# GadGadGad/Convolutional-KAN-for-Image-Classification

Hardware: AMD Instinct MI355X
Metric: images/sec fwd+bwd KAN-VGG11 3x32x32 bs=256/GPU (higher is better)
Workload: dtype f32

## Files before the change

convolutional-kan-for-image-classification_amd/_lib.py:

```python
from __future__ import annotations

import ctypes as C
import os
from typing import Optional

_HERE = os.path.dirname(os.path.abspath(__file__))
LIB_PATH = os.environ.get("KANCONV_LIB") or os.path.join(_HERE, "libkanconv.so")

KAN_MAX_PLANES = 16
KAN_MAX_TABLE = 32
KAN_FP_WORDS = 192
BASIS_BSPLINE, BASIS_RBF, BASIS_CHEBY, BASIS_POLY, BASIS_FOURIER, BASIS_RELU, BASIS_GRAM = 0, 1, 2, 3, 4, 5, 6
ACT_NONE, ACT_IDENTITY, ACT_GELU, ACT_SILU, ACT_RELU, ACT_TANH, ACT_SIGMOID, ACT_GELU_TANH = -1, 0, 1, 2, 3, 4, 5, 6
ORDER_QUAD_FWD, ORDER_ROWBLK8_FWD, ORDER_QUAD_BWD_DATA, ORDER_FWD_WEIGHT_SIDE = 1, 2, 4, 8


class KanGeom(C.Structure):
    _fields_ = [(n, C.c_int) for n in ("B", "C", "H", "W", "O", "Ho", "Wo", "kh", "kw", "sh", "sw", "ph", "pw", "dh", "dw", "groups")] + \
               [("x_bstride", C.c_longlong), ("y_bstride", C.c_longlong)]


class KanBasis(C.Structure):
    _fields_ = [("kind", C.c_int), ("n_basis", C.c_int), ("order", C.c_int), ("act", C.c_int),
                ("p0", C.c_float), ("p1", C.c_float), ("table", C.c_float * KAN_MAX_TABLE), ("chan_table", C.c_void_p)]


class KanPlan(C.Structure):
    _fields_ = [(n, C.c_int) for n in ("P", "K", "IPC", "KC", "Kpad", "Opad", "fwd_splits", "bwd_data_splits", "bwd_weight_splits",
                                          "fwd_target", "bwd_data_target", "bwd_weight_target", "x_pm_wanted", "dz_pm_wanted", "bwd_weight_expanded", "row_blocks", "e_pm_wanted", "fwd_expanded", "fwd_halo", "bwd_weight_halo",
                                          "fwd_band", "bwd_weight_band")] + \
               [(n, C.c_longlong) for n in ("packed_weight_bytes", "bwd_data_weight_bytes", "fwd_slab_elems", "bwd_data_slab_elems",
                                            "bwd_weight_slab_elems", "e_pm_elems")]


class KanNormRoute(C.Structure):
    _fields_ = [(n, C.c_int) for n in ("kernel", "G", "EPL", "PPI", "NT", "pool", "lds", "held", "blocks", "strided")]


NORM_GENERIC, NORM_REGS = 0, 1
NORM_POOL_NONE, NORM_POOL_2X2, NORM_POOL_K = 0, 1, 2


class KanWavGeom(C.Structure):
    _fields_ = [(n, C.c_int) for n in ("B", "C", "H", "W", "O", "Ho", "Wo", "kh", "kw", "sh", "sw", "ph", "pw", "dh", "dw", "wavelet")] + \
               [("x_bstride", C.c_longlong), ("u_bstride", C.c_longlong)]


class KanWavRoute(C.Structure):
    _fields_ = [(n, C.c_int) for n in ("TH", "TW", "NIMG", "RH", "RW", "tiles_h", "tiles_w", "fwd_shrunk", "fwd_nimg_cut", "fwd_lds_bytes", "fwd_fits",
                                       "fwd_blocks", "bwd_input_kernel", "bwd_input_blocks", "params_kernel", "passes", "chunks", "BH", "NI", "RU",
                                       "CU", "XP", "UP", "bands", "items", "items_per_chunk", "lds_bytes", "px_per_chunk")]


WAV_BI_TAPS9, WAV_BI_STRIDE1, WAV_BI_STRIDED = 0, 1, 2
WAV_PAR_TILED, WAV_PAR_PIXEL = 0, 1


WAVELETS = {"mexican_hat": 0, "morlet": 1, "dog": 2, "meyer": 3, "shannon": 4}

_P, _I, _LL, _F, _D = C.c_void_p, C.c_int, C.c_longlong, C.c_float, C.c_double
_GP, _BP = C.POINTER(KanGeom), C.POINTER(KanBasis)
SIGNATURES = {
    "kan_version": (C.c_char_p, []),
    "kan_last_error": (C.c_char_p, []),
    "kan_plan": (_I, [_GP, _BP, C.POINTER(KanPlan)]),
    "kan_tile_orders": (_I, [_GP, _BP]),
    "kan_pack_weights": (_I, [_P, _P, _P, _P, _GP, _BP, _P]),
    "kan_pack_weights_iod": (_I, [_P, _P, _P, _GP, _BP, _P]),
    "kan_pack_cacheable": (_I, [_GP, _BP]),
    "kan_pack_weights_cached": (_I, [_P, _P, _P, _P, _GP, _BP, _P, _I, _I, _I, _P]),
    "kan_conv_fwd": (_I, [_P, _P, _P, _P, _GP, _BP, _P, _P]),
    "kan_position_major": (_I, [_P, _P, _I, _I, _I, _LL, _P]),
    "kan_conv_bwd_data": (_I, [_P, _P, _P, _P, _P, _P, _GP, _BP, _P, _P]),
    "kan_conv_bwd_data_params": (_I, [_P, _P, _P, _P, _P, _P, _P, _GP, _BP, _P, _P]),
    "kan_conv_bwd_weight": (_I, [_P, _P, _P, _P, _GP, _BP, _P, _P, _P]),
    "kan_position_major_expanded": (_I, [_P, _P, _GP, _BP, _P]),
    "kan_conv_fwd_expanded": (_I, [_P, _P, _P, _GP, _BP, _P]),
    "kan_conv_fwd_expanded_order": (_I, [_P, _P, _P, _GP, _BP, _P, _I]),
    "kan_conv_bwd_weight_expanded": (_I, [_P, _P, _P, _GP, _BP, _P]),
    "kan_unpack_wgrad": (_I, [_P, _P, _P, _GP, _BP, _P]),
    "kan_unpack_wgrad_iod": (_I, [_P, _P, _GP, _BP, _P]),
    "kan_slab_reduce": (_I, [_P, _I, _LL, _P, _I, _I, _I, _LL, _P]),
    "kan_instnorm_prelu_fwd": (_I, [_P, _I, _LL, _P, _P, _P, _P, _P, _P, _P, _I, _I, _I, _LL, _F, _I, _P]),
    "kan_instnorm_prelu_bwd": (_I, [_P, _P, _P, _P, _P, _P, _P, _P, _P, _P, _P, _I, _I, _I, _LL, _I, _P]),
    "kan_instnorm_prelu_pool_fwd": (_I, [_P, _I, _LL, _P, _P, _P, _P, _P, _P, _P, _P, _I, _I, _I, _I, _LL, _F, _I, _P]),
    "kan_instnorm_prelu_pool_bwd": (_I, [_P, _P, _P, _P, _P, _P, _P, _P, _P, _P, _P, _P, _I, _I, _I, _I, _LL, _I, _P]),
    "kan_instnorm_prelu_poolk_fwd": (_I, [_P, _I, _LL, _P, _P, _P, _P, _P, _P, _P, _P, _I, _I, _I, _I, _LL, _F, _I, _I, _I, _P]),
    "kan_instnorm_prelu_poolk_bwd": (_I, [_P, _P, _P, _P, _P, _P, _P, _P, _P, _P, _P, _P, _I, _I, _I, _I, _LL, _I, _I, _I, _P]),
    "kan_norm_route": (_I, [_I, _I, _I, _I, _I, _LL, _I, _LL, _I, _I, _I, _I, C.POINTER(KanNormRoute)]),
    "kan_batchnorm_workspace_bytes": (_LL, [_I, _I]),
    "kan_batchnorm_prelu_fwd": (_I, [_P, _I, _LL, _P, _P, _P, _P, _P, _P, _P, _P, _P, _P, _P, _I, _I, _I, _I, _LL, _F, _D, _I, _I, _P]),
    "kan_batchnorm_prelu_bwd": (_I, [_P, _P, _P, _P, _P, _P, _P, _P, _P, _P, _P, _P, _P, _I, _I, _I, _I, _LL, _I, _I, _P]),
    "kan_split_supported": (_I, [C.POINTER(KanGeom), C.POINTER(KanBasis)]),
    "kan_split_weight_bytes": (_LL, [C.POINTER(KanGeom), C.POINTER(KanBasis)]),
    "kan_split_pack_weights": (_I, [_P, _P, _P, C.POINTER(KanGeom), C.POINTER(KanBasis), _P]),
    "kan_conv_fwd_split": (_I, [_P, _P, _P, C.POINTER(KanGeom), C.POINTER(KanBasis), _P]),
    "kan_split_bwd_data_weight_bytes": (_LL, [C.POINTER(KanGeom), C.POINTER(KanBasis)]),
    "kan_split_pack_weights_bwd_data": (_I, [_P, _P, _P, C.POINTER(KanGeom), C.POINTER(KanBasis), _P]),
    "kan_conv_bwd_data_split": (_I, [_P, _P, _P, _P, C.POINTER(KanGeom), C.POINTER(KanBasis), _P]),
    "kan_split_bwd_weight_workspace_bytes": (_LL, [C.POINTER(KanGeom), C.POINTER(KanBasis)]),
    "kan_conv_bwd_weight_split": (_I, [_P, _P, _P, _P, _P, C.POINTER(KanGeom), C.POINTER(KanBasis), _P]),
    "kan_wav_fwd": (_I, [_P, _P, _P, _P, _P, C.POINTER(KanWavGeom), _P]),
    "kan_wav_bwd_input": (_I, [_P, _P, _P, _P, _P, _P, C.POINTER(KanWavGeom), _P]),
    "kan_wav_param_workspace": (_LL, [C.POINTER(KanWavGeom)]),
    "kan_wav_bwd_params": (_I, [_P, _P, _P, _P, _P, _P, _P, _P, _P, C.POINTER(KanWavGeom), _P]),
    "kan_wav_route": (_I, [C.POINTER(KanWavGeom), C.POINTER(KanWavRoute)]),
    "kan_adamw_step": (_I, [_P, _P, _P, _P, _LL, _D, _D, _D, _D, _D, _I, _F, _P]),
    "kan_adamw_step_segments": (_I, [_P, _P, _P, _P, _P, _P, _P, _P, _P, _I, _I, _D, _D, _D, _D, _D, _I, _F, _P]),
    "kan_adamw_advance": (_I, [_P, _P, _I, _P]),
    "kan_adamw_step_segments_dev": (_I, [_P, _P, _P, _P, _P, _P, _P, _P, _P, _P, _I, _I, _D, _D, _D, _D, _F, _P]),
    "kan_adamw_dev_args": (_I, [_P, _P, _D, _D, _D, _D, _F, _P, _P]),
    "kan_grad_sqnorm_chunks": (_I, [_P, _P, _P, _P, _I, _I, _P, _P]),
# ... 48 lines not shown
```

convolutional-kan-for-image-classification_amd/csrc/kan_internal.h:

```cpp
#pragma once
#include <type_traits>
#include "kanconv.h"

int kan_fail_msg(const char* fmt, const char* a);
int kan_raise_lds_limit(const void* kernel, int bytes);

enum : int {
    FAST_GENERIC = 0,
    FAST_BSPLINE_SILU = 1,
    FAST_BSPLINE_GELU = 2,
    FAST_RBF8 = 3,
    FAST_CHEBY5 = 4,
    FAST_CHEBY4 = 5,
    FAST_POLY4 = 6,
    FAST_POLY3 = 7,
    FAST_RBF5 = 8,
    FAST_RELU8 = 9,
    FAST_GRAM4 = 10,
    FAST_POLY1 = 11,
    FAST_LAST = 11
};
enum : unsigned {
    ON_TAP_MAJOR = 1u << 0,
    ON_BIG_TILES = 1u << 1,
// ... 76 lines not shown
    unsigned char ph_a[KAN_BAND_MAX_PHASES], ph_b[KAN_BAND_MAX_PHASES];
    short ph_tap0[KAN_BAND_MAX_PHASES + 1];
    unsigned short tap_shift[KAN_BAND_MAX_TAPS];
    unsigned short tap_rt[KAN_BAND_MAX_TAPS];
    short tap_step[KAN_BAND_MAX_TAPS], tap_nt[KAN_BAND_MAX_TAPS];
} KanBandCfg;

void kan_band_cfg(const KanGeom* g, const KanBasis* b, int fast, KanBandCfg* cfg);
int kan_band_bwd_weight_launch(const float* dz, const float* x, const float* xn, float* dwp, const KanGeom* g, const KanBasis* b,
                               const KanBandCfg* cfg, int splits, long long slab_elems, void* stream);
int kan_band_fwd_launch(const float* x, const float* xn, const float* wp, float* z, const KanGeom* g, const KanBasis* b,
                        const KanBandCfg* cfg, int splits, long long slab_elems, void* stream);

constexpr int DW_T = 9;
constexpr int DW_MAX_TP = 96;

enum class Route { TAP_MAJOR, DW, BAND, HALO, EXPANDED };

struct FwdCfg { int TO, TP, tiles_o, tiles_p, chunks, splits, slots; };
struct BdCfg { int CH, tiles_c, tiles_p, n_ob, Opad32, chunks, splits; };
struct BwCfg { int TR, TO, tiles_r, tiles_o, chunks, splits, slots; };
struct BwHaloCfg { int R, nimg, spb, n_bands, tiles_r, tiles_o, splits, bands_per_split; };

struct ConvPlan {
    KanPlan pub;
    int fast;
    Route fwd, bwd_data, bwd_weight;
    bool pm_fwd, pm_bwd_data, pm_bwd_weight;
    bool rowblk_bwd_data;
    bool quad_fwd;
    bool quad_bd;
    bool rowblk8_fwd;
    bool fwd_wq;
    bool pmdma_xcd, pm_lpt, pm_xcd;
    FwdCfg fc;
    BdCfg bd;
    BwCfg bw;
    BwHaloCfg bwh;
    KanBandCfg band;
};
int plan_conv(const KanGeom* g, const KanBasis* b, ConvPlan* cp);

int live_taps_out(const KanGeom* g, int hw);
int live_taps_in(const KanGeom* g, int hw);
int live_positions_for_tap(const KanGeom* g, int tap);
int balance_tiles(const int* weight, int n, unsigned short* idx);
```

convolutional-kan-for-image-classification_amd/csrc/kan_plan.hip:

```cpp
#include <hip/hip_runtime.h>
#include <cstdio>
#include <cstdlib>
#include <cstring>
#include "kanconv.h"
#include "kan_device.h"
#include "kan_common.h"
#include "kan_internal.h"

namespace {

int fail(const char* msg) { return kan_fail_msg("%s", msg); }

int check(const KanGeom* g, const KanBasis* b) {
    if (!g || !b) return fail("null geometry/basis");
    if (g->groups < 0 || g->groups > 65535) return fail("groups out of range");
    if (g->B <= 0 || g->C <= 0 || g->O <= 0 || g->H <= 0 || g->W <= 0 || g->Ho <= 0 || g->Wo <= 0) return fail("non-positive dimension");
    if (g->kh <= 0 || g->kw <= 0 || g->sh <= 0 || g->sw <= 0 || g->dh <= 0 || g->dw <= 0 || g->ph < 0 || g->pw < 0) return fail("bad conv parameters");
    if (g->kh > 255 || g->kw > 255 || g->C > 65535) return fail("kernel size / channel count out of supported range");
    if ((g->H + 2 * g->ph - g->dh * (g->kh - 1) - 1) / g->sh + 1 != g->Ho || (g->W + 2 * g->pw - g->dw * (g->kw - 1) - 1) / g->sw + 1 != g->Wo)
        return fail("Ho/Wo inconsistent with H/W, kernel, stride, padding, dilation");
    if ((long long)g->B * g->Ho * g->Wo >= (1ll << 31) || (long long)g->B * g->H * g->W >= (1ll << 31)) return fail("pixel count exceeds int32");
    if ((long long)g->B * g->x_bstride * 4 >= (1ll << 31) || (long long)g->B * g->y_bstride * 4 >= (1ll << 31))
        return fail("activation tensors must be smaller than 2 GiB (32-bit buffer offsets)");
    if (g->x_bstride < (long long)ngroups(g) * g->C * g->H * g->W || g->y_bstride < (long long)ngroups(g) * g->O * g->Ho * g->Wo)
// ... 310 lines not shown
        const bool use18 = (long long)i18 * pl->P * 16 > (long long)i16 * pl->P * 18;
        pl->KC = use18 ? 18 : 16;
        pl->IPC = use18 ? i18 : i16;
        if (pl->P >= 10 && pl->P <= 12) { pl->KC = 12; pl->IPC = 1; }
        if (halo) { pl->KC = 2 * pl->P; pl->IPC = 2; }
    }
    pl->Kpad = ceil_div(g->C * T, pl->IPC) * pl->KC;
    if (band) { pl->KC = c.band.NPLE; pl->IPC = c.band.NG; pl->Kpad = c.band.n_steps * c.band.NPLE; }
    pl->Opad = round_up(g->O, 64);
    pl->packed_weight_bytes = (long long)G * pl->Kpad * pl->Opad * 4;
    c.bd = bd_cfg(g, *pl);
    pl->bwd_data_weight_bytes = (long long)G * T * c.bd.Opad32 * c.bd.tiles_c * 128 * 4;
    pl->fwd_slab_elems = (long long)g->B * g->y_bstride;
    pl->bwd_data_slab_elems = (long long)g->B * g->x_bstride;
    pl->bwd_weight_slab_elems = (long long)G * pl->K * pl->Opad;
    const bool big = big_tiles(f, *pl);
    c.fc = fwd_cfg(g, *pl, big, c.pm_fwd, halo);
    c.bw = bw_cfg(g, *pl, big, c.pm_bwd_weight);
    if (halo_bw) c.bwh = bw_halo_cfg(g, *pl);
    pl->fwd_splits = band ? c.band.fwd_splits : c.fc.splits;
    pl->bwd_data_splits = c.bd.splits;
    pl->bwd_weight_splits = halo_bw ? c.bwh.splits : c.bw.splits;
    if (band_bw) {
        pl->bwd_weight_splits = c.band.bw_splits;
        pl->bwd_weight_slab_elems = (long long)G * pl->Kpad * pl->Opad;
    }
    pl->fwd_target = pl->bwd_data_target = pl->bwd_weight_target = 0;
    const bool rowblk_fwd = halo && g->H == 4 && g->W == 4 && c.fc.TO == 256;
    c.quad_fwd = rowblk_fwd && g->B % 32 == 0 && !tuning_off("KAN_QUAD_FWD");
    c.quad_bd = c.rowblk_bwd_data && g->B % 32 == 0 && !tuning_off("KAN_QUAD_BD");
    c.rowblk8_fwd = halo && g->H == 8 && g->W == 8 && c.fc.TO == 256 && g->B % 4 == 0 && !tuning_off("KAN_ROWBLK8_FWD");
    c.fwd_wq = c.fwd == Route::EXPANDED && g->H == 2 && g->W == 2 && g->Ho == 2 && g->Wo == 2 && g->kh == 3 && g->kw == 3 && g->sh == 1 && g->sw == 1 &&
               g->ph == 1 && g->pw == 1 && g->dh == 1 && g->dw == 1 && pl->P == 9 && pl->KC == 18 && g->y_bstride % 4 == 0 && !tuning_off("KAN_PMDMA_FWD_WQ");
    if (dw) {
        pl->fwd_splits = pl->bwd_data_splits = 1;
        pl->bwd_weight_splits = dw_weight_chunks(g);
        pl->bwd_data_weight_bytes = pl->packed_weight_bytes;
        c.pm_fwd = c.pm_bwd_data = c.pm_bwd_weight = false;
    }
    if (c.pm_fwd) {
        LiveClass cls[16]; const int plane = g->Ho * g->Wo;
        const long long tiles_per_pos = (long long)ceil_div(g->B, c.fc.TP) * c.fc.tiles_o * G;
        for (int hw = 0; hw < plane; ++hw) cls[hw] = LiveClass{tiles_per_pos, live_taps_out(g, hw) * ceil_div(g->C, pl->IPC)};
        pl->fwd_target = pick_target_steps(cls, plane, 8, 4.0 * g->B * g->O * g->Ho * g->Wo * G, &pl->fwd_splits, c.fc.slots);
    }
    if (c.pm_bwd_weight) {
        LiveClass cw[32];
        const long long tiles_per_tap = (long long)ceil_div((long long)g->C * pl->P, c.bw.TR) * c.bw.tiles_o * G;
        for (int tap = 0; tap < T; ++tap) cw[tap] = LiveClass{tiles_per_tap, live_positions_for_tap(g, tap) * ceil_div(g->B, 16)};
        pl->bwd_weight_target = pick_target_steps(cw, T, 16, 4.0 * pl->K * pl->Opad * G, &pl->bwd_weight_splits, c.bw.slots);
    }
    if (c.pm_bwd_data) {
        LiveClass cls[16]; const int plane = g->H * g->W;
        const long long tiles_per_pos = (long long)ceil_div(g->B, 128) * c.bd.tiles_c * G;
        for (int hw = 0; hw < plane; ++hw) cls[hw] = LiveClass{tiles_per_pos, live_taps_in(g, hw) * c.bd.n_ob};
        pl->bwd_data_target = pick_target_steps(cls, plane, 8, 4.0 * g->B * g->C * g->H * g->W * G, &pl->bwd_data_splits);
    }
    pl->fwd_halo = c.fwd == Route::HALO;
    pl->fwd_band = c.fwd == Route::BAND;
    pl->fwd_expanded = c.fwd == Route::EXPANDED;
    pl->bwd_weight_halo = c.bwd_weight == Route::HALO;
    pl->bwd_weight_band = c.bwd_weight == Route::BAND;
    pl->bwd_weight_expanded = c.bwd_weight == Route::EXPANDED;
    pl->x_pm_wanted = (c.pm_fwd && c.fwd != Route::EXPANDED) || (c.pm_bwd_weight && c.bwd_weight != Route::EXPANDED);
    pl->dz_pm_wanted = c.pm_bwd_data || c.pm_bwd_weight;
    pl->e_pm_wanted = pl->fwd_expanded || pl->bwd_weight_expanded;
// ... 5 lines not shown
```

convolutional-kan-for-image-classification_amd/csrc/kanconv.hip:

```cpp
#include <hip/hip_runtime.h>
#include <cstdio>
#include <cstdlib>
#include <cstring>
#include <cmath>
#include <cstdint>
#include <mutex>
#include <type_traits>
#include <vector>
#include "kanconv.h"
#include "kan_device.h"

#include "kan_common.h"
#include "kan_internal.h"

namespace {


thread_local char g_err[512] = "";
int fail(const char* fmt, const char* a = "") {
    snprintf(g_err, sizeof(g_err), fmt, a);
    return -1;
}
}
int kan_fail_msg(const char* fmt, const char* a) { return fail(fmt, a); }
// ... 1281 lines not shown
    for (int cur = 0; ch < ch1; cur ^= 1) {
        stage(cur);
        __syncthreads();
        ch = next_live(ch + 1);
        if (ch < ch1) issue(ch);
        const float* cE = sE + cur * (KPX * LDE) + MRG;
        const float* cZ = sZ + cur * (KPX * LDZ);
        const unsigned ae = lds_addr(cE + kh2 * LDE + ar), az = lds_addr(cZ + kh2 * LDZ + bo);
        KAN_MFMA_STEP(KPX / 2, ae, LDE, az, LDZ);
    }

    float* out = dwp + (size_t)blk.z * slab_elems;
#pragma unroll
    for (int mi = 0; mi < 2; ++mi)
#pragma unroll
        for (int r = 0; r < 16; ++r) {
            const int row = k0 + w_r * 64 + mi * 32 + mfma_row(r, lane);
            if (row >= Krows) continue;
#pragma unroll
            for (int ni = 0; ni < 2; ++ni) {
                const int o = o_tile0 + w_c * 64 + ni * 32 + (lane & 31);
                out[(size_t)row * Opad + o] = acc[mi][ni][r];
            }
        }
}

#define LDS_READ4W(r0, r1, r2, r3, a0, a1, b, oA, oB0, oB1)                                                              \
    asm volatile("ds_read_b32 %0, %4 offset:%7\n\tds_read_b32 %1, %5 offset:%7\n\tds_read_b32 %2, %6 offset:%8\n\tds_read_b32 %3, %6 offset:%9" \
                 : "=&v"(r0), "=&v"(r1), "=&v"(r2), "=&v"(r3) : "v"(a0), "v"(a1), "v"(b), "n"(oA), "n"(oB0), "n"(oB1) : "memory")

template <int FAST, int W, int R, int NIMG>
__global__ __launch_bounds__(256, 4) void k_conv_bwd_weight_halo(
    const float* __restrict__ dz, const float* __restrict__ x, float* __restrict__ dwp, DevGeom g, DevBasis bs, int Krows, int Opad,
    int n_bands, int bands_per_split, long long slab_elems, unsigned x_bytes, unsigned dz_bytes, int tiles_o) {
    constexpr int KIND = fast_kind(FAST);
    constexpr int P = fast_planes(FAST), T = 9, PT = P * T;
    constexpr int TR = 128, TO = 128, NT = 256, KPX = 16;
    constexpr int HWc = W + 2, HIMG = (R + 2) * HWc, CELLS = NIMG * HIMG;
    constexpr int PS = W == 16 ? CELLS + 1 : W == 8 ? CELLS + 3 : W == 4 ? CELLS + 7 : CELLS + 1;
    constexpr int NCH = (TR + PT - 2) / PT + 1;
    constexpr int HB = NCH * P * PS;
    constexpr int BP = NIMG * R * W, SPB = BP / KPX;
    constexpr int ZB = KPX * TO;
    constexpr int NU = NCH * NIMG * (R + 2) * W;
    constexpr int SLOTS = (NU + NT - 1) / NT;
    static_assert(BP % KPX == 0 && SPB % 2 == 0 && SPB >= SLOTS + 1 && PS > CELLS && (NIMG == 1 || R == W), "band shape");
    __shared__ float sH[2 * HB];
    __shared__ __attribute__((aligned(16))) float sZ[2 * ZB];
    __shared__ float sTab[KAN_MAX_TABLE];

    const int tid = threadIdx.x, lane = tid & 63;
    const int wave = __builtin_amdgcn_readfirstlane(tid >> 6);
    const int w_r = wave >> 1, w_c = wave & 1, kh2 = lane >> 5;
    const int HoWo = g.Ho * g.Wo, HW = g.H * g.W;
    const BlockId blk = xcd_block_order(true);
    const int grp = blk.y / tiles_o;
    const int k0 = blk.x * TR, o_tile0 = (blk.y - grp * tiles_o) * TO;
    x += (size_t)grp * g.C * HW;
    dz += (size_t)grp * g.O * HoWo;
    dwp += (size_t)grp * Krows * Opad;
    const int c0 = k0 / PT;

    if (tid < KAN_MAX_TABLE) sTab[tid] = bs.tab[tid];
    for (int i = tid; i < 2 * HB; i += NT) sH[i] = 0.f;
    float* const dump = sH + CELLS;

    int u_src[SLOTS], u_dst[SLOTS], u_hr[SLOTS], u_ch[SLOTS]; unsigned u_ok = 0;
#pragma unroll
    for (int k = 0; k < SLOTS; ++k) {
        const int idx = tid + k * NT;
        constexpr int UPC = NIMG * (R + 2) * W, UPI = (R + 2) * W;
        const int ch = idx / UPC, ri = idx - ch * UPC, img = ri / UPI, rc = ri - img * UPI, hr = rc / W, col = rc - hr * W;
        u_src[k] = (c0 + ch) * HW + img * (int)g.xbs + (hr - 1) * W + col;
        u_dst[k] = ch * (P * PS) + img * HIMG + hr * HWc + col + 1;
        u_hr[k] = hr - 1; u_ch[k] = c0 + ch;
        u_ok |= ((idx < NU && c0 + ch < g.C) ? 1u : 0u) << k;
    }
    const kan_rsrc x_rs = make_rsrc(x, x_bytes), dz_rs = make_rsrc(dz, dz_bytes);

    unsigned aA[2];
#pragma unroll
    for (int mi = 0; mi < 2; ++mi) {
        int row = k0 + w_r * 64 + mi * 32 + (lane & 31);
        if (row >= Krows) row = k0;
        const int c = row / PT, rem = row - c * PT, tap = rem / P, pl_ = rem - tap * P, r = tap / 3, t = tap - 3 * r;
        aA[mi] = lds_addr(sH + ((c - c0) * P + pl_) * PS + r * HWc + t + kh2);
    }
    unsigned bB[KPX / 2];
    {
        const int ol = w_c * 64 + (lane & 31), sw = (ol >> 1) & 15;
#pragma unroll
        for (int kk = 0; kk < KPX / 2; ++kk) bB[kk] = lds_addr(sZ + ol * KPX + ((2 * kk + kh2) ^ sw));
    }
    unsigned zoff[8];
#pragma unroll
    for (int j = 0; j < 8; ++j) {
        const int ol = 4 * (wave * 8 + j) + (lane >> 4), q = (lane & 15) ^ ((ol >> 1) & 15);
        zoff[j] = o_tile0 + ol < g.O ? (unsigned)((o_tile0 + ol) * HoWo + q) * 4u : KAN_OOB;
    }
    constexpr int BPI = NIMG > 1 ? 1 : (W * W) / BP;
    auto issue_dz = [&](int band, int st, int zb) {
        const int gpx = band * BP + st * KPX;
        const int b = gpx / (W * W), px0 = gpx - b * (W * W);
        const int soff = __builtin_amdgcn_readfirstlane((b * (int)g.ybs + px0) * 4);
        float* dst = sZ + zb * ZB + wave * (8 * 64);
#pragma unroll
        for (int j = 0; j < 8; ++j)
            __builtin_amdgcn_raw_ptr_buffer_load_lds(dz_rs, (__attribute__((address_space(3))) void*)(dst + j * 64), 4, (int)zoff[j], soff, 0, 0);
    };
    float xv[SLOTS]; unsigned inb_mask = 0;
    auto load_band = [&](int band) {
        const int b = NIMG > 1 ? band * NIMG : band / BPI, h0 = NIMG > 1 ? 0 : (band - b * BPI) * R;
        const int sbase = b * (int)g.xbs + h0 * W;
        inb_mask = 0;
#pragma unroll
        for (int k = 0; k < SLOTS; ++k) {
// ... 19 lines not shown
    __syncthreads();
    if (nb0 < nb1) {
        load_band(nb0);
#pragma unroll
        for (int k = 0; k < SLOTS; ++k) expand(k, 0);
        issue_dz(nb0, 0, 0);
    }
    int hb = 0;
    for (int band = nb0; band < nb1; ++band, hb ^= 1) {
        const unsigned hoff = (unsigned)(hb * HB * 4);
        const unsigned a0 = aA[0] + hoff, a1 = aA[1] + hoff;
#pragma unroll
        for (int st = 0; st < SPB; ++st) {
            asm volatile("s_waitcnt vmcnt(0)" ::: "memory");
            __syncthreads();
            if (st + 1 < SPB) issue_dz(band, st + 1, (st + 1) & 1);
            else if (band + 1 < nb1) issue_dz(band + 1, 0, 0);
            if (st == 0) { if (band + 1 < nb1) load_band(band + 1); }
            else if (st - 1 < SLOTS) { if (band + 1 < nb1) expand(st - 1, hb ^ 1); }
            float fa[2][2], fb[2][2];
#define KAN_OFFA(kk) ((((16 * st + 2 * (kk)) / (R * W)) * HIMG + (((16 * st + 2 * (kk)) % (R * W)) / W) * HWc + ((16 * st + 2 * (kk)) % W)) * 4)
#define KAN_OFFB(kk) (((st & 1) * ZB) * 4)
            LDS_READ4W(fa[0][0], fa[0][1], fb[0][0], fb[0][1], a0, a1, bB[0], KAN_OFFA(0), KAN_OFFB(0), KAN_OFFB(0) + 32 * KPX * 4);
#pragma unroll
            for (int kk = 0; kk < KPX / 2; ++kk) {
                const int c_ = kk & 1, n_ = c_ ^ 1;
                if (kk + 1 < KPX / 2) {
                    LDS_READ4W(fa[n_][0], fa[n_][1], fb[n_][0], fb[n_][1], a0, a1, bB[kk + 1], KAN_OFFA(kk + 1), KAN_OFFB(kk + 1),
                               KAN_OFFB(kk + 1) + 32 * KPX * 4);
                    LDS_WAIT4(fa[c_][0], fa[c_][1], fb[c_][0], fb[c_][1], 4);
                } else {
                    LDS_WAIT4(fa[c_][0], fa[c_][1], fb[c_][0], fb[c_][1], 0);
                }
                acc[0][0] = MFMA32(fa[c_][0], fb[c_][0], acc[0][0]);
                acc[0][1] = MFMA32(fa[c_][0], fb[c_][1], acc[0][1]);
                acc[1][0] = MFMA32(fa[c_][1], fb[c_][0], acc[1][0]);
                acc[1][1] = MFMA32(fa[c_][1], fb[c_][1], acc[1][1]);
            }
#undef KAN_OFFA
#undef KAN_OFFB
        }
    }

    float* out = dwp + (size_t)blk.z * slab_elems;
#pragma unroll
    for (int mi = 0; mi < 2; ++mi)
#pragma unroll
        for (int r = 0; r < 16; ++r) {
            const int row = k0 + w_r * 64 + mi * 32 + mfma_row(r, lane);
            if (row >= Krows) continue;
#pragma unroll
            for (int ni = 0; ni < 2; ++ni) {
                const int o = o_tile0 + w_c * 64 + ni * 32 + (lane & 31);
                out[(size_t)row * Opad + o] = acc[mi][ni][r];
            }
        }
}

template <int KIND, int FAST>
__global__ __launch_bounds__(256) void k_expand_pm(const float* __restrict__ x, float* __restrict__ e_pm, DevBasis bs, int B, int CHW, int HW, int Cg,
                                                   long long bstride, float* __restrict__ dump) {
    __shared__ float tile[32][33];
    __shared__ float sTab[KAN_MAX_TABLE];
    const int e0 = blockIdx.x * 32, b0 = blockIdx.y * 32;
    const int tx = threadIdx.x & 31, ty = threadIdx.x >> 5;
    const int P = FAST ? fast_planes(FAST) : bs.P;
    if (threadIdx.x < KAN_MAX_TABLE) sTab[threadIdx.x] = bs.tab[threadIdx.x];
#pragma unroll
    for (int i = 0; i < 4; ++i) {
        const int b = b0 + ty + 8 * i, e = e0 + tx;
        tile[ty + 8 * i][tx] = (b < B && e < CHW) ? x[(size_t)b * bstride + e] : 0.f;
    }
    __syncthreads();
#pragma unroll
    for (int i = 0; i < 4; ++i) {
        const int e = e0 + ty + 8 * i, b = b0 + tx;
        if (e < CHW && b < B) {
            const float v = tile[tx][ty + 8 * i];
            stage_unit<KIND, FAST>(bs, sTab, true, v, v, e_pm + (size_t)e * P * B + b, B, dump + threadIdx.x, (e / HW) % Cg);
        }
    }
}
// ... 1233 lines not shown
    if (iod) {
        const IodLaunch l = iod_launch(g, pl);
        hipLaunchKernelGGL(k_pack_iod, dim3(l.blocks), dim3(256), 0, st, w_basis, wp, q, l.o_tiles, l.n_tiles, iod_vec(w_basis, wp, g, b));
    } else {
        hipLaunchKernelGGL(k_pack, grid, dim3(256), 0, st, w_base, w_basis, wp, q, nb_base, wp_gs, tiles_x, tiles_y, fp, fp_cur);
    }
    if (wd && cp.bwd_data == Route::DW) {
        if (hipMemcpyAsync(wd, wp, (size_t)pl.packed_weight_bytes, hipMemcpyDeviceToDevice, st) != hipSuccess) return fail("memcpy failed");
    } else if (wd) {
        const BdCfg& c = cp.bd;
        const int bx = c.tiles_c * 4, by = c.Opad32 / 32 * G;
        const long long nt = (long long)bx * by;
        const long long capd = fp ? 128 : 1024;
        dim3 gd((unsigned)(nt < capd ? nt : capd), 1, T);
        hipLaunchKernelGGL(k_pack_bwd_data, gd, dim3(256), 0, st, (const float*)wp, wd, q, c.CH, c.tiles_c, c.Opad32, wp_gs, bx, by, fp, fp_cur);
    }
    return launch_ok("pack");
}

int kan_pack_weights(const float* w_base, const float* w_basis, float* wp, float* wd, const KanGeom* g, const KanBasis* b, void* stream) {
    return pack_weights_impl(w_base, w_basis, wp, wd, g, b, nullptr, 0, stream);
}

int kan_pack_weights_iod(const float* coeffs, float* wp, float* wd, const KanGeom* g, const KanBasis* b, void* stream) {
    if (int rc = iod_scope(g, b)) return rc;
    return pack_weights_impl(nullptr, coeffs, wp, wd, g, b, nullptr, 0, stream, true);
}

int kan_tile_orders(const KanGeom* g, const KanBasis* b) {
    ConvPlan cp;
    if (plan_conv(g, b, &cp)) return 0;
    const bool halo = cp.fwd == Route::HALO;
    return (halo && cp.quad_fwd ? KAN_ORDER_QUAD_FWD : 0) | (halo && cp.rowblk8_fwd ? KAN_ORDER_ROWBLK8_FWD : 0) | (cp.quad_bd ? KAN_ORDER_QUAD_BWD_DATA : 0) |
           (cp.fwd_wq ? KAN_ORDER_FWD_WEIGHT_SIDE : 0);
}

int kan_pack_cacheable(const KanGeom* g, const KanBasis* b) {
    ConvPlan cp;
    if (plan_conv(g, b, &cp)) return 0;
    if ((long long)g->O * g->C * (b->n_basis + 1) * g->kh * g->kw >= (1ll << 31)) return 0;
    return (!pack_needs_clear(g, cp.pub) && cp.fwd != Route::DW && ngroups(g) == 1) ? 1 : 0;
}

int kan_pack_weights_cached(const float* w_base, const float* w_basis, float* wp, float* wd, const KanGeom* g, const KanBasis* b,
                            unsigned long long* ring, int cur, int force, int sample_stride, void* stream) {
    static_assert(KAN_FP_WORDS == 3 * FP_LANES, "ring size");
    if (!ring || cur < 0 || cur > 2 || sample_stride < 1) return fail("bad fingerprint ring arguments");
    if (!kan_pack_cacheable(g, b)) return fail("cached packing is not offered for this geometry (kan_pack_cacheable)");
    const int hb = b->act != KAN_ACT_NONE;
    if ((hb && !w_base) || !w_basis) return fail("null weight pointer");
    if (((size_t)w_basis & 15) || (hb && ((size_t)w_base & 15))) return fail("cached packing needs 16-byte aligned weight tensors");
    const int T = g->kh * g->kw;
    const long long na = hb ? (long long)g->O * g->C * T : 0, nbs = (long long)g->O * g->C * b->n_basis * T;
    const long long groups4 = ((na + 3) / 4 + (nbs + 3) / 4 + sample_stride - 1) / sample_stride;
    long long blocks = (groups4 + 256 * 8 - 1) / (256 * 8); if (blocks > 4096) blocks = 4096; if (blocks < 1) blocks = 1;
    hipLaunchKernelGGL(k_fingerprint, dim3((unsigned)blocks), dim3(256), 0, (hipStream_t)stream, hb ? w_base : w_basis, (unsigned)na, w_basis,
                       (unsigned)nbs, (unsigned)sample_stride, ring, cur);
    if (int rc = launch_ok("fingerprint")) return rc;
    return pack_weights_impl(w_base, w_basis, wp, wd, g, b, force ? nullptr : ring, cur, stream);
}

static int unpack_wgrad_impl(const float* dwp, float* dw_base, float* dw_basis, const KanGeom* g, const KanBasis* b, void* stream, bool iod) {
    ConvPlan cp;
    if (int rc = plan_conv(g, b, &cp)) return rc;
    const KanPlan& pl = cp.pub;
    const int hb = b->act != KAN_ACT_NONE;
    if ((hb && !dw_base) || !dw_basis || !dwp) return fail("null weight-gradient pointer");
// ... 164 lines not shown
    DevGeom dg = dev_geom(g);
    dg.pix_major = (dz_pm && cp.pm_bwd_data) ? 1 : 0;
    if (dg.pix_major) dz = dz_pm;
    DevBasis db = dev_basis(b);
    if ((long long)c.tiles_c * ngroups(g) > 65535) return fail("groups * channel tiles exceed the grid limit");
    dim3 grid(c.tiles_p, c.tiles_c * ngroups(g), pl.bwd_data_splits);
    const int cps = dg.pix_major ? pl.bwd_data_target : ceil_div(c.chunks, pl.bwd_data_splits);
    TilePerm perm; perm.n = 0;
    if (dg.pix_major) perm = tile_perm(c.tiles_p, [&](int t) {
        const int hw = (int)(((long long)t * 128) / g->B);
        return ceil_div(live_taps_in(g, hw < g->H * g->W ? hw : 0) * c.n_ob, cps > 0 ? cps : 1);
    });
    const int fast = (fast_spec(cp.fast).xn_bwd ? (x != xn && dxn) : (x == xn && !dxn)) ? cp.fast : FAST_GENERIC;
    const bool rb = !dg.pix_major && cp.rowblk_bwd_data;
    const bool quad = rb && cp.quad_bd && dz_pm && x == xn && !dxn;
    const unsigned dz_bytes = (unsigned)((long long)g->B * g->y_bstride * 4);
    auto launch = [&](auto kind, auto fast, auto rbv) {
        hipLaunchKernelGGL((k_conv_bwd_data<decltype(kind)::value, decltype(fast)::value, decltype(rbv)::value>), grid, dim3(256), 0, st,
                           decltype(rbv)::value == 2 ? dz_pm : dz, x, xn, wd,
                           dx, dxn, dg, db, c.CH, c.tiles_c, c.n_ob, c.Opad32, c.chunks, cps, pl.bwd_data_slab_elems, dz_bytes, perm, dpar);
    };
    const bool launched = dispatch_fast<ON_TAP_MAJOR>(fast, [&](auto fv) {
        constexpr int F = decltype(fv)::value;
        if constexpr (fast_has(F, ON_ROWBLK_BWD_DATA)) {
            if (quad) return launch(IC<fast_kind(F)>{}, fv, IC<2>{});
            if (rb) return launch(IC<fast_kind(F)>{}, fv, IC<1>{});
        }
        launch(IC<fast_kind(F)>{}, fv, IC<0>{});
    });
    if (!launched) dispatch_kind(b->kind, [&](auto kind) { launch(kind, IC<FAST_GENERIC>{}, IC<0>{}); });
    return launch_ok("conv_bwd_data");
}

int kan_conv_bwd_weight(const float* dz, const float* x, const float* xn, float* dwp, const KanGeom* g, const KanBasis* b,
                        const float* x_pm, const float* dz_pm, void* stream) {
    ConvPlan cp;
    if (int rc = plan_conv(g, b, &cp)) return rc;
    const KanPlan& pl = cp.pub;
    if (!dz || !x || !xn || !dwp) return fail("null tensor pointer");
    if ((b->kind == KAN_BASIS_RELU || b->kind == KAN_BASIS_GRAM) && !b->chan_table) return fail("ReLU / Gram bases need their device parameter table (chan_table)");
    hipStream_t st = (hipStream_t)stream;
    if (cp.bwd_weight == Route::DW) {
        DevGeom dgd = dev_geom(g); DevBasis dbd = dev_basis(b);
        dim3 grid(pl.bwd_weight_splits, ngroups(g));
        dispatch_kind(b->kind, [&](auto kind) {
            hipLaunchKernelGGL((k_dw_bwd_weight<decltype(kind)::value>), grid, dim3(256), 0, st, dz, x, xn, dwp, dgd, dbd, pl.K, pl.Opad, pl.bwd_weight_slab_elems);
        });
        return launch_ok("dw_bwd_weight");
    }
    if (cp.bwd_weight == Route::BAND) {
        if (x != xn && !fast_spec(cp.fast).xn_fwd) return fail("this basis / activation pair runs on single-input kernels: pass xn == x");
        return kan_band_bwd_weight_launch(dz, x, xn, dwp, g, b, &cp.band, pl.bwd_weight_splits, pl.bwd_weight_slab_elems, stream);
    }
    const unsigned x_bytes = (unsigned)((long long)g->B * g->x_bstride * 4), dz_bytes = (unsigned)((long long)g->B * g->y_bstride * 4);
    if (cp.bwd_weight == Route::HALO) {
        if (x != xn) return fail("internal: the channel-major weight-gradient layout needs x == xn");
        const BwHaloCfg& hc = cp.bwh;
        const DevGeom dgh = dev_geom(g); const DevBasis dbh = dev_basis(b);
        if ((long long)hc.tiles_o * ngroups(g) > 65535) return fail("groups * output tiles exceed the grid limit");
        dim3 grid(hc.tiles_r, hc.tiles_o * ngroups(g), hc.splits);
        dispatch_fast<ON_HALO_BWD_WEIGHT>(cp.fast, [&](auto fv) {
            auto launch = [&](auto w, auto r, auto nimg) {
                hipLaunchKernelGGL((k_conv_bwd_weight_halo<decltype(fv)::value, decltype(w)::value, decltype(r)::value, decltype(nimg)::value>), grid,
                                   dim3(256), 0, st, dz, x, dwp, dgh, dbh, pl.K, pl.Opad, hc.n_bands, hc.bands_per_split, pl.bwd_weight_slab_elems,
                                   x_bytes, dz_bytes, hc.tiles_o);
            };
            if (g->W == 16) launch(IC<16>{}, IC<4>{}, IC<1>{});
            else if (g->W == 8) launch(IC<8>{}, IC<8>{}, IC<1>{});
            else launch(IC<4>{}, IC<4>{}, IC<2>{});
        });
        return launch_ok("conv_bwd_weight_halo");
    }
    const BwCfg& c = cp.bw;
    DevGeom dg = dev_geom(g);
    dg.pix_major = (x_pm && dz_pm && x == xn && cp.pm_bwd_weight) ? 1 : 0;
    if (dg.pix_major) { x = x_pm; xn = x_pm; dz = dz_pm; }
    DevBasis db = dev_basis(b);
    if ((long long)c.tiles_o * ngroups(g) > 65535) return fail("groups * output tiles exceed the grid limit");
    dim3 grid(c.tiles_r, c.tiles_o * ngroups(g), pl.bwd_weight_splits);
    const int cps = dg.pix_major ? pl.bwd_weight_target : ceil_div(c.chunks, pl.bwd_weight_splits);
    if (x != xn && !fast_spec(cp.fast).xn_fwd)
        return fail("this basis / activation pair runs on single-input kernels: pass xn == x");
    auto launch = [&](auto kind, auto fast, auto wr, auto wc) {
        constexpr int WR = decltype(wr)::value, WC = decltype(wc)::value;
        hipLaunchKernelGGL((k_conv_bwd_weight<decltype(kind)::value, decltype(fast)::value, WR, WC>), grid, dim3(WR * WC * 64), 0, st, dz, x, xn, dwp,
                           dg, db, pl.K, pl.Opad, c.chunks, cps, pl.bwd_weight_slab_elems, x_bytes, dz_bytes, c.tiles_o);
    };
    auto tiles = [&](auto kind, auto fast) {
        if (c.TO == 128) launch(kind, fast, IC<2>{}, IC<2>{});
        else launch(kind, fast, IC<4>{}, IC<1>{});
    };
    const bool fast = dispatch_fast<ON_TAP_MAJOR>(cp.fast, [&](auto fv) {
        constexpr int F = decltype(fv)::value;
        if constexpr (fast_has(F, ON_BIG_TILES)) {
            if (c.TO == 256) return launch(IC<fast_kind(F)>{}, fv, IC<2>{}, IC<4>{});
        }
        tiles(IC<fast_kind(F)>{}, fv);
    });
    if (!fast) dispatch_kind(b->kind, [&](auto kind) { tiles(kind, IC<FAST_GENERIC>{}); });
    return launch_ok("conv_bwd_weight");
}

int kan_position_major_expanded(const float* x, float* e_pm, const KanGeom* g, const KanBasis* b, void* stream) {
    ConvPlan cp;
    if (int rc = plan_conv(g, b, &cp)) return rc;
    const KanPlan& pl = cp.pub;
    if (!x || !e_pm) return fail("null tensor pointer");
    if (!pl.e_pm_wanted) return fail("this geometry / basis does not use the expanded position-major copy (plan.e_pm_wanted)");
    const int G = ngroups(g), CHW = G * g->C * g->H * g->W;
    DevBasis db = dev_basis(b);
    dim3 grid(ceil_div(CHW, 32), ceil_div(g->B, 32));
    float* dump = e_pm + (pl.e_pm_elems - 256);
    if ((b->kind == KAN_BASIS_RELU || b->kind == KAN_BASIS_GRAM) && !b->chan_table) return fail("ReLU / Gram bases need their device parameter table (chan_table)");
    dispatch_fast<ON_EXPANDED>(cp.fast, [&](auto fv) {
        constexpr int F = decltype(fv)::value;
        hipLaunchKernelGGL((k_expand_pm<fast_kind(F), F>), grid, dim3(256), 0, (hipStream_t)stream, x, e_pm, db, g->B, CHW, g->H * g->W, g->C, g->x_bstride, dump);
    });
    return launch_ok("position_major_expanded");
}

static int conv_fwd_expanded_impl(const float* e_pm, const float* wp, float* z, const KanGeom* g, const KanBasis* b, void* stream, int order) {
    ConvPlan cp;
    if (int rc = plan_conv(g, b, &cp)) return rc;
    const KanPlan& pl = cp.pub;
    if (!e_pm || !wp || !z) return fail("null tensor pointer");
    if (cp.fwd != Route::EXPANDED) return fail("the forward of this geometry / basis does not read the expanded position-major copy (plan.fwd_expanded)");
    if (order >= 0 && order != 0 && order != KAN_ORDER_FWD_WEIGHT_SIDE) return fail("order must be 0 or KAN_ORDER_FWD_WEIGHT_SIDE");
    if (order == KAN_ORDER_FWD_WEIGHT_SIDE && !cp.fwd_wq) return fail("this geometry does not offer the weight-side order (kan_tile_orders)");
    const FwdCfg& c = cp.fc;
    DevGeom dg = dev_geom(g);
    dg.pix_major = 1;
    if ((long long)c.tiles_o * ngroups(g) > 65535) return fail("groups * output tiles exceed the grid limit");
    if (order < 0 ? cp.fwd_wq : order != 0) {
        if ((size_t)z & 15) return fail("the weight-side forward stores 16-byte groups: z must be 16-byte aligned");
        dim3 grid(c.tiles_p, c.tiles_o * ngroups(g), pl.fwd_splits);
// ... 293 lines not shown
```

include/kanconv.h:

```cpp
#ifndef KANCONV_H
#define KANCONV_H

#ifdef __cplusplus
extern "C" {
#endif

#define KAN_MAX_PLANES 16
#define KAN_MAX_TABLE  32
#define KAN_FP_WORDS   192

enum { KAN_BASIS_BSPLINE = 0, KAN_BASIS_RBF = 1, KAN_BASIS_CHEBY = 2, KAN_BASIS_POLY = 3, KAN_BASIS_FOURIER = 4, KAN_BASIS_RELU = 5, KAN_BASIS_GRAM = 6 };
enum { KAN_ACT_NONE = -1, KAN_ACT_IDENTITY = 0, KAN_ACT_GELU = 1, KAN_ACT_SILU = 2, KAN_ACT_RELU = 3,
       KAN_ACT_TANH = 4, KAN_ACT_SIGMOID = 5, KAN_ACT_GELU_TANH = 6 };

typedef struct KanGeom {
    int B, C, H, W;
    int O, Ho, Wo;
    int kh, kw, sh, sw, ph, pw, dh, dw;
    int groups;
    long long x_bstride;
    long long y_bstride;
} KanGeom;

#define KAN_ORDER_PACK(mode, first) ((int)(mode) | ((int)(first) << 8))
// ... 8 lines not shown

typedef struct KanPlan {
    int P;
    int K;
    int IPC, KC;
    int Kpad, Opad;
    int fwd_splits;
    int bwd_data_splits;
    int bwd_weight_splits;
    int fwd_target, bwd_data_target, bwd_weight_target;
    int x_pm_wanted, dz_pm_wanted;
    int bwd_weight_expanded;
    int row_blocks;
    int e_pm_wanted, fwd_expanded;
    int fwd_halo, bwd_weight_halo;
    int fwd_band, bwd_weight_band;
    long long packed_weight_bytes;
    long long bwd_data_weight_bytes;
    long long fwd_slab_elems;
    long long bwd_data_slab_elems;
    long long bwd_weight_slab_elems;
    long long e_pm_elems;
} KanPlan;

const char* kan_version(void);
const char* kan_last_error(void);

int kan_plan(const KanGeom* geom, const KanBasis* basis, KanPlan* plan);

#define KAN_ORDER_QUAD_FWD 1
#define KAN_ORDER_ROWBLK8_FWD 2
#define KAN_ORDER_QUAD_BWD_DATA 4
#define KAN_ORDER_FWD_WEIGHT_SIDE 8
int kan_tile_orders(const KanGeom* geom, const KanBasis* basis);

int kan_pack_weights(const float* w_base, const float* w_basis, float* wp, float* wd,
                     const KanGeom* geom, const KanBasis* basis, void* stream);

int kan_pack_weights_iod(const float* coeffs, float* wp, float* wd, const KanGeom* geom, const KanBasis* basis, void* stream);

int kan_pack_cacheable(const KanGeom* geom, const KanBasis* basis);
int kan_pack_weights_cached(const float* w_base, const float* w_basis, float* wp, float* wd,
                            const KanGeom* geom, const KanBasis* basis, unsigned long long* ring, int cur, int force,
                            int sample_stride, void* stream);

int kan_conv_fwd(const float* x, const float* xn, const float* wp, float* z,
                 const KanGeom* geom, const KanBasis* basis, const float* x_pm, void* stream);

int kan_position_major(const float* src, float* dst, int B, int Cn, int HW, long long bstride, void* stream);

int kan_conv_bwd_data(const float* dz, const float* x, const float* xn, const float* wd,
                      float* dx, float* dxn,
                      const KanGeom* geom, const KanBasis* basis, const float* dz_pm, void* stream);

int kan_conv_bwd_data_params(const float* dz, const float* x, const float* xn, const float* wd, float* dx, float* dxn, float* dparams,
                             const KanGeom* geom, const KanBasis* basis, const float* dz_pm, void* stream);

int kan_conv_bwd_weight(const float* dz, const float* x, const float* xn, float* dwp,
                        const KanGeom* geom, const KanBasis* basis, const float* x_pm, const float* dz_pm, void* stream);

int kan_position_major_expanded(const float* x, float* e_pm, const KanGeom* geom, const KanBasis* basis, void* stream);
int kan_conv_fwd_expanded(const float* e_pm, const float* wp, float* z, const KanGeom* geom, const KanBasis* basis, void* stream);
int kan_conv_fwd_expanded_order(const float* e_pm, const float* wp, float* z, const KanGeom* geom, const KanBasis* basis, void* stream, int order);
int kan_conv_bwd_weight_expanded(const float* dz_pm, const float* e_pm, float* dwp,
                                 const KanGeom* geom, const KanBasis* basis, void* stream);

int kan_unpack_wgrad(const float* dwp, float* dw_base, float* dw_basis,
                     const KanGeom* geom, const KanBasis* basis, void* stream);

int kan_unpack_wgrad_iod(const float* dwp, float* dcoeffs, const KanGeom* geom, const KanBasis* basis, void* stream);

int kan_slab_reduce(const float* slabs, int n_slabs, long long slab_elems, float* out,
                    int B, int Cn, int HW, long long bstride, void* stream);

int kan_instnorm_prelu_fwd(const float* z, int n_slabs, long long slab_elems, float* z_out,
                           const float* gamma, const float* beta, const float* prelu_a,
                           float* y, float* mean, float* rstd,
                           int B, int Cn, int HW, long long bstride, float eps, int prelu_span, void* stream);

int kan_instnorm_prelu_bwd(const float* dy, const float* z, const float* mean, const float* rstd,
                           const float* gamma, const float* beta, const float* prelu_a,
                           float* dz, float* dgamma, float* dbeta, float* dprelu,
                           int B, int Cn, int HW, long long bstride, int prelu_span, void* stream);

int kan_instnorm_prelu_pool_fwd(const float* z, int n_slabs, long long slab_elems, float* z_out,
                                const float* gamma, const float* beta, const float* prelu_a,
                                float* y_pooled, unsigned char* pool_idx, float* mean, float* rstd,
                                int B, int Cn, int H, int W, long long bstride, float eps, int prelu_span, void* stream);
int kan_instnorm_prelu_pool_bwd(const float* dy_pooled, const unsigned char* pool_idx, const float* z, const float* mean, const float* rstd,
                                const float* gamma, const float* beta, const float* prelu_a,
                                float* dz, float* dgamma, float* dbeta, float* dprelu,
                                int B, int Cn, int H, int W, long long bstride, int prelu_span, void* stream);
// ... 122 lines not shown
```

Baseline: 18120.

## Reorder bwd-weight halo tile rows by tap row to skip dead MFMAs

For the W=8 halo backward-weight kernel with a whole image per block, the K rows of each tile are permuted so rows with the same tap row (top/middle/bottom) sit together. Wave sub-tiles made entirely of top-row taps skip their MFMAs for the first output row, and those made of bottom-row taps skip them for the last row, because padding makes those products zero. The output rows are remapped through a shared-memory table at write-back, and a new ordered entry point plus tile-orders flag exposes the mode. The cost is extra index math, two more barriers and divergent MFMA guards.

```diff
diff --git a/convolutional-kan-for-image-classification_amd/_lib.py b/convolutional-kan-for-image-classification_amd/_lib.py
--- a/convolutional-kan-for-image-classification_amd/_lib.py
+++ b/convolutional-kan-for-image-classification_amd/_lib.py
@@ -12,7 +12,7 @@
 KAN_FP_WORDS = 192
 BASIS_BSPLINE, BASIS_RBF, BASIS_CHEBY, BASIS_POLY, BASIS_FOURIER, BASIS_RELU, BASIS_GRAM = 0, 1, 2, 3, 4, 5, 6
 ACT_NONE, ACT_IDENTITY, ACT_GELU, ACT_SILU, ACT_RELU, ACT_TANH, ACT_SIGMOID, ACT_GELU_TANH = -1, 0, 1, 2, 3, 4, 5, 6
-ORDER_QUAD_FWD, ORDER_ROWBLK8_FWD, ORDER_QUAD_BWD_DATA, ORDER_FWD_WEIGHT_SIDE = 1, 2, 4, 8
+ORDER_QUAD_FWD, ORDER_ROWBLK8_FWD, ORDER_QUAD_BWD_DATA, ORDER_FWD_WEIGHT_SIDE, ORDER_BWD_WEIGHT_TAPROW = 1, 2, 4, 8, 16
 
 
 class KanGeom(C.Structure):
@@ -78,6 +78,7 @@
     "kan_conv_fwd_expanded": (_I, [_P, _P, _P, _GP, _BP, _P]),
     "kan_conv_fwd_expanded_order": (_I, [_P, _P, _P, _GP, _BP, _P, _I]),
     "kan_conv_bwd_weight_expanded": (_I, [_P, _P, _P, _GP, _BP, _P]),
+    "kan_conv_bwd_weight_order": (_I, [_P, _P, _P, _GP, _BP, _P, _I]),
     "kan_unpack_wgrad": (_I, [_P, _P, _P, _GP, _BP, _P]),
     "kan_unpack_wgrad_iod": (_I, [_P, _P, _GP, _BP, _P]),
     "kan_slab_reduce": (_I, [_P, _I, _LL, _P, _I, _I, _I, _LL, _P]),
diff --git a/convolutional-kan-for-image-classification_amd/csrc/kan_internal.h b/convolutional-kan-for-image-classification_amd/csrc/kan_internal.h
--- a/convolutional-kan-for-image-classification_amd/csrc/kan_internal.h
+++ b/convolutional-kan-for-image-classification_amd/csrc/kan_internal.h
@@ -132,6 +132,7 @@
     bool quad_bd;
     bool rowblk8_fwd;
     bool fwd_wq;
+    bool bw_taprow;
     bool pmdma_xcd, pm_lpt, pm_xcd;
     FwdCfg fc;
     BdCfg bd;
diff --git a/convolutional-kan-for-image-classification_amd/csrc/kan_plan.hip b/convolutional-kan-for-image-classification_amd/csrc/kan_plan.hip
--- a/convolutional-kan-for-image-classification_amd/csrc/kan_plan.hip
+++ b/convolutional-kan-for-image-classification_amd/csrc/kan_plan.hip
@@ -366,6 +366,7 @@
     c.rowblk8_fwd = halo && g->H == 8 && g->W == 8 && c.fc.TO == 256 && g->B % 4 == 0 && !tuning_off("KAN_ROWBLK8_FWD");
     c.fwd_wq = c.fwd == Route::EXPANDED && g->H == 2 && g->W == 2 && g->Ho == 2 && g->Wo == 2 && g->kh == 3 && g->kw == 3 && g->sh == 1 && g->sw == 1 &&
                g->ph == 1 && g->pw == 1 && g->dh == 1 && g->dw == 1 && pl->P == 9 && pl->KC == 18 && g->y_bstride % 4 == 0 && !tuning_off("KAN_PMDMA_FWD_WQ");
+    c.bw_taprow = c.bwd_weight == Route::HALO && g->W == 8 && !tuning_off("KAN_BW_TAPROW");
     if (dw) {
         pl->fwd_splits = pl->bwd_data_splits = 1;
         pl->bwd_weight_splits = dw_weight_chunks(g);
diff --git a/convolutional-kan-for-image-classification_amd/csrc/kanconv.hip b/convolutional-kan-for-image-classification_amd/csrc/kanconv.hip
--- a/convolutional-kan-for-image-classification_amd/csrc/kanconv.hip
+++ b/convolutional-kan-for-image-classification_amd/csrc/kanconv.hip
@@ -1337,9 +1337,9 @@
 template <int FAST, int W, int R, int NIMG>
 __global__ __launch_bounds__(256, 4) void k_conv_bwd_weight_halo(
     const float* __restrict__ dz, const float* __restrict__ x, float* __restrict__ dwp, DevGeom g, DevBasis bs, int Krows, int Opad,
-    int n_bands, int bands_per_split, long long slab_elems, unsigned x_bytes, unsigned dz_bytes, int tiles_o) {
+    int n_bands, int bands_per_split, long long slab_elems, unsigned x_bytes, unsigned dz_bytes, int tiles_o, int taprow) {
     constexpr int KIND = fast_kind(FAST);
-    constexpr int P = fast_planes(FAST), T = 9, PT = P * T;
+    constexpr int P = fast_planes(FAST), T = 9, PT = P * T, P3 = 3 * P;
     constexpr int TR = 128, TO = 128, NT = 256, KPX = 16;
     constexpr int HWc = W + 2, HIMG = (R + 2) * HWc, CELLS = NIMG * HIMG;
     constexpr int PS = W == 16 ? CELLS + 1 : W == 8 ? CELLS + 3 : W == 4 ? CELLS + 7 : CELLS + 1;
@@ -1365,6 +1365,27 @@
     dz += (size_t)grp * g.O * HoWo;
     dwp += (size_t)grp * Krows * Opad;
     const int c0 = k0 / PT;
+    constexpr bool WHOLE = NIMG == 1 && R == W;
+    const bool tr = WHOLE && taprow;
+    auto cnt = [&](int k, int r) { const int q = k / PT; return q * P3 + min(max(k - q * PT - r * P3, 0), P3); };
+    const int k1 = min(k0 + TR, Krows);
+    int t_f[3], t_e[4];
+    t_e[0] = 0;
+#pragma unroll
+    for (int r = 0; r < 3; ++r) { t_f[r] = cnt(k0, r); t_e[r + 1] = t_e[r] + cnt(k1, r) - t_f[r]; }
+    auto tile_row = [&](int i) -> int {
+        if (!tr || i >= t_e[3]) return k0 + i;
+        const int r = i < t_e[1] ? 0 : i < t_e[2] ? 1 : 2;
+        const int j = t_f[r] + i - t_e[r], q = j / P3;
+        return q * PT + r * P3 + (j - q * P3);
+    };
+    bool top_dead[2], bot_dead[2];
+#pragma unroll
+    for (int mi = 0; mi < 2; ++mi) {
+        const int s0 = w_r * 64 + mi * 32;
+        top_dead[mi] = tr && s0 + 32 <= t_e[1];
+        bot_dead[mi] = tr && s0 >= t_e[2] && s0 + 32 <= t_e[3];
+    }
 
     if (tid < KAN_MAX_TABLE) sTab[tid] = bs.tab[tid];
     for (int i = tid; i < 2 * HB; i += NT) sH[i] = 0.f;
@@ -1386,7 +1407,7 @@
     unsigned aA[2];
 #pragma unroll
     for (int mi = 0; mi < 2; ++mi) {
-        int row = k0 + w_r * 64 + mi * 32 + (lane & 31);
+        int row = tile_row(w_r * 64 + mi * 32 + (lane & 31));
         if (row >= Krows) row = k0;
         const int c = row / PT, rem = row - c * PT, tap = rem / P, pl_ = rem - tap * P, r = tap / 3, t = tap - 3 * r;
         aA[mi] = lds_addr(sH + ((c - c0) * P + pl_) * PS + r * HWc + t + kh2);
@@ -1472,10 +1493,17 @@
                 } else {
                     LDS_WAIT4(fa[c_][0], fa[c_][1], fb[c_][0], fb[c_][1], 0);
                 }
-                acc[0][0] = MFMA32(fa[c_][0], fb[c_][0], acc[0][0]);
-                acc[0][1] = MFMA32(fa[c_][0], fb[c_][1], acc[0][1]);
-                acc[1][0] = MFMA32(fa[c_][1], fb[c_][0], acc[1][0]);
-                acc[1][1] = MFMA32(fa[c_][1], fb[c_][1], acc[1][1]);
+                constexpr int RW = R * W;
+                const int brow = ((16 * st + 2 * kk) % RW) / W;
+                const bool top = WHOLE && brow == 0, bot = WHOLE && brow == R - 1;
+                if (!((top && top_dead[0]) || (bot && bot_dead[0]))) {
+                    acc[0][0] = MFMA32(fa[c_][0], fb[c_][0], acc[0][0]);
+                    acc[0][1] = MFMA32(fa[c_][0], fb[c_][1], acc[0][1]);
+                }
+                if (!((top && top_dead[1]) || (bot && bot_dead[1]))) {
+                    acc[1][0] = MFMA32(fa[c_][1], fb[c_][0], acc[1][0]);
+                    acc[1][1] = MFMA32(fa[c_][1], fb[c_][1], acc[1][1]);
+                }
             }
 #undef KAN_OFFA
 #undef KAN_OFFB
@@ -1483,11 +1511,17 @@
     }
 
     float* out = dwp + (size_t)blk.z * slab_elems;
+    int* const sRow = reinterpret_cast<int*>(sZ);
+    if constexpr (WHOLE) {
+        __syncthreads();
+        if (tid < TR) sRow[tid] = tile_row(tid);
+        __syncthreads();
+    }
 #pragma unroll
     for (int mi = 0; mi < 2; ++mi)
 #pragma unroll
         for (int r = 0; r < 16; ++r) {
-            const int row = k0 + w_r * 64 + mi * 32 + mfma_row(r, lane);
+            const int pos = w_r * 64 + mi * 32 + mfma_row(r, lane), row = WHOLE ? sRow[pos] : k0 + pos;
             if (row >= Krows) continue;
 #pragma unroll
             for (int ni = 0; ni < 2; ++ni) {
@@ -2787,7 +2821,7 @@
     if (plan_conv(g, b, &cp)) return 0;
     const bool halo = cp.fwd == Route::HALO;
     return (halo && cp.quad_fwd ? KAN_ORDER_QUAD_FWD : 0) | (halo && cp.rowblk8_fwd ? KAN_ORDER_ROWBLK8_FWD : 0) | (cp.quad_bd ? KAN_ORDER_QUAD_BWD_DATA : 0) |
-           (cp.fwd_wq ? KAN_ORDER_FWD_WEIGHT_SIDE : 0);
+           (cp.fwd_wq ? KAN_ORDER_FWD_WEIGHT_SIDE : 0) | (cp.bw_taprow ? KAN_ORDER_BWD_WEIGHT_TAPROW : 0);
 }
 
 int kan_pack_cacheable(const KanGeom* g, const KanBasis* b) {
@@ -3018,12 +3052,17 @@
     return launch_ok("conv_bwd_data");
 }
 
-int kan_conv_bwd_weight(const float* dz, const float* x, const float* xn, float* dwp, const KanGeom* g, const KanBasis* b,
-                        const float* x_pm, const float* dz_pm, void* stream) {
+static int conv_bwd_weight_impl(const float* dz, const float* x, const float* xn, float* dwp, const KanGeom* g, const KanBasis* b,
+                                const float* x_pm, const float* dz_pm, void* stream, int order) {
     ConvPlan cp;
     if (int rc = plan_conv(g, b, &cp)) return rc;
     const KanPlan& pl = cp.pub;
     if (!dz || !x || !xn || !dwp) return fail("null tensor pointer");
+    if (order >= 0) {
+        if (order != 0 && order != KAN_ORDER_BWD_WEIGHT_TAPROW) return fail("order must be 0 or KAN_ORDER_BWD_WEIGHT_TAPROW");
+        if (!(cp.bwd_weight == Route::HALO && g->W == 8))
+            return fail("this geometry does not offer the tap-row order (kan_tile_orders)");
+    }
     if ((b->kind == KAN_BASIS_RELU || b->kind == KAN_BASIS_GRAM) && !b->chan_table) return fail("ReLU / Gram bases need their device parameter table (chan_table)");
     hipStream_t st = (hipStream_t)stream;
     if (cp.bwd_weight == Route::DW) {
@@ -3049,7 +3088,7 @@
             auto launch = [&](auto w, auto r, auto nimg) {
                 hipLaunchKernelGGL((k_conv_bwd_weight_halo<decltype(fv)::value, decltype(w)::value, decltype(r)::value, decltype(nimg)::value>), grid,
                                    dim3(256), 0, st, dz, x, dwp, dgh, dbh, pl.K, pl.Opad, hc.n_bands, hc.bands_per_split, pl.bwd_weight_slab_elems,
-                                   x_bytes, dz_bytes, hc.tiles_o);
+                                   x_bytes, dz_bytes, hc.tiles_o, (order < 0 ? cp.bw_taprow : order != 0) ? 1 : 0);
             };
             if (g->W == 16) launch(IC<16>{}, IC<4>{}, IC<1>{});
             else if (g->W == 8) launch(IC<8>{}, IC<8>{}, IC<1>{});
@@ -3087,6 +3126,16 @@
     return launch_ok("conv_bwd_weight");
 }
 
+int kan_conv_bwd_weight(const float* dz, const float* x, const float* xn, float* dwp, const KanGeom* g, const KanBasis* b,
+                        const float* x_pm, const float* dz_pm, void* stream) {
+    return conv_bwd_weight_impl(dz, x, xn, dwp, g, b, x_pm, dz_pm, stream, -1);
+}
+
+int kan_conv_bwd_weight_order(const float* dz, const float* x, float* dwp, const KanGeom* g, const KanBasis* b, void* stream, int order) {
+    if (order < 0) return fail("order must be 0 or KAN_ORDER_BWD_WEIGHT_TAPROW");
+    return conv_bwd_weight_impl(dz, x, x, dwp, g, b, nullptr, nullptr, stream, order);
+}
+
 int kan_position_major_expanded(const float* x, float* e_pm, const KanGeom* g, const KanBasis* b, void* stream) {
     ConvPlan cp;
     if (int rc = plan_conv(g, b, &cp)) return rc;
diff --git a/include/kanconv.h b/include/kanconv.h
--- a/include/kanconv.h
+++ b/include/kanconv.h
@@ -64,6 +64,7 @@
 #define KAN_ORDER_ROWBLK8_FWD 2
 #define KAN_ORDER_QUAD_BWD_DATA 4
 #define KAN_ORDER_FWD_WEIGHT_SIDE 8
+#define KAN_ORDER_BWD_WEIGHT_TAPROW 16
 int kan_tile_orders(const KanGeom* geom, const KanBasis* basis);
 
 int kan_pack_weights(const float* w_base, const float* w_basis, float* wp, float* wd,
@@ -90,6 +91,8 @@
 
 int kan_conv_bwd_weight(const float* dz, const float* x, const float* xn, float* dwp,
                         const KanGeom* geom, const KanBasis* basis, const float* x_pm, const float* dz_pm, void* stream);
+
+int kan_conv_bwd_weight_order(const float* dz, const float* x, float* dwp, const KanGeom* geom, const KanBasis* basis, void* stream, int order);
 
 int kan_position_major_expanded(const float* x, float* e_pm, const KanGeom* geom, const KanBasis* basis, void* stream);
 int kan_conv_fwd_expanded(const float* e_pm, const float* wp, float* z, const KanGeom* geom, const KanBasis* basis, void* stream);
```

Result: no change. 18200, median of 6 (+0.4%).
